# bad-samaritan/Polmux

Measured on AMD Instinct MI355X. Metric: dual-pol Gsample/s through SSFM+Rx-DSP, higher is better.
Workload: dtype f64

## Files before the change

### include/polmux_hip.h

```cpp
#ifndef POLMUX_HIP_H
#define POLMUX_HIP_H

#include <stddef.h>
#include <stdint.h>

#ifdef __cplusplus
extern "C" {
#endif

#define PLX_OK 0
#define PLX_ERR_HIP (-1)
#define PLX_ERR_ARG (-2)
#define PLX_ERR_UNSUPPORTED (-3)
#define PLX_ERR_REFERENCE (-4)
#define PLX_ERR_TIMEOUT (-5)

const char *plx_last_error(void);
int plx_abi_version(void);
int plx_device_count(int *count);
int plx_set_device(int device);

int plx_release_all(void);
int plx_gateway_stats(int64_t *out);
int plx_gateway_stats_ex(int64_t *out, int n);
// ... 6 lines not shown
    int32_t nfc;
    int32_t dual_pol;
    int32_t max_frames;
    int32_t fls[4];
    double dzmaxt;
    double dphimaxt;
    double alphalin;
    double length;
    int32_t nplates;
    int32_t manakov;
    const double *gam;
    const double *betat;
    const double *db1;
} plx_ssfm_desc;

typedef struct plx_ssfm plx_ssfm;

int plx_ssfm_create(plx_ssfm **plan, const plx_ssfm_desc *desc);
#define PLX_SSFM_SHARE_DEVICE 1u
#define PLX_SSFM_XPM_MANAKOV 2u
int plx_ssfm_create_ex(plx_ssfm **plan, const plx_ssfm_desc *desc, uint32_t flags);
typedef struct plx_ssfm_tuning {
    uint32_t size;
    int32_t no_fuse;
    int32_t short_rows;
    int32_t no_row_split;
    int32_t p1, logW;
    int32_t col_threads;
    int32_t rowr;
    int32_t rowsm;
    int32_t row256_split, row4k_split, rowg_split;
    int32_t no_pmd_tab;
    int32_t store_late;
    int32_t row_rev;
    int32_t safe_landing;
    int32_t reserved_[4];
    double barrier_timeout_ms;
} plx_ssfm_tuning;
int plx_ssfm_tuning_defaults(plx_ssfm_tuning *tuning);
int plx_ssfm_tuning_override(const plx_ssfm_tuning *tuning);
int plx_ssfm_create_tuned(plx_ssfm **plan, const plx_ssfm_desc *desc, uint32_t flags, const plx_ssfm_tuning *tuning);
int plx_ssfm_destroy(plx_ssfm *plan);
int plx_ssfm_set_birefringence(plx_ssfm *plan, const double *db0, const double *theta,
                               const double *epsilon, int nsets);
int plx_ssfm_set_birefringence_dev(plx_ssfm *plan, const double *db0, const double *theta,
                                   const double *epsilon, int nsets, void *stream);
int plx_ssfm_propagate_dev(plx_ssfm *plan, double *d_ux, double *d_uy, int nframes, void *stream);
int plx_ssfm_set_step_sequence(plx_ssfm *plan, const double *dz, int nsteps);
int plx_ssfm_log_steps(plx_ssfm *plan, int max_steps);
int plx_ssfm_step_sequence(plx_ssfm *plan, int frame, double *dz, int max_steps);
int plx_ssfm_results(plx_ssfm *plan, int nframes, double *firstdz, int32_t *ncycle);
int plx_ssfm_stats(plx_ssfm *plan, int64_t *row_pass_launches, int64_t *sample_steps);
int plx_ssfm_utilisation(plx_ssfm *plan, int64_t *frame_steps, int64_t *slots_listed, int64_t *slots_launched);
int plx_ssfm_info(plx_ssfm *plan, int32_t *info);
int plx_ssfm_barrier_timeouts(plx_ssfm *plan, int32_t *count, int rearm);
int plx_ssfm_profile(plx_ssfm *plan, int enable);
int plx_ssfm_kernel_times(plx_ssfm *plan, double *ms, int64_t *launches);

int plx_matrix_ssfm(double *uxr, double *uxi, double *uyr, double *uyi, const plx_ssfm_desc *desc,
                    const double *db0, const double *theta, const double *epsilon,
                    double *firstdz, int32_t *ncycle);
int plx_scalar_ssfm(double *ur, double *ui, const plx_ssfm_desc *desc, double *firstdz, int32_t *ncycle);
int plx_scalar_ssfm_adaptive(double *ur, double *ui, const plx_ssfm_desc *desc, int tolflag, double ltol,
                             double safety, double *firstdz, int32_t *ncycle, int32_t *nrej);

typedef struct plx_cde plx_cde;
int plx_cde_create(plx_cde **plan, int64_t fft_len, int64_t L, const double *H_interleaved);
int plx_cde_create_wdm(plx_cde **plan, int64_t fft_len, int64_t L, const double *H_interleaved, int32_t nch,
                       int32_t rows_per_channel);
int plx_cde_destroy(plx_cde *plan);
int plx_cde_apply_dev(plx_cde *plan, const double *d_x, double *d_y, int64_t nx, int nsig, void *stream);
int plx_cde_ofde(const double *xr, const double *xi, const double *yr, const double *yi, int64_t nx,
                 double fs, double lambda_ref, double span, double D, double S, int64_t fft_len,
                 int64_t L, double *oxr, double *oxi, double *oyr, double *oyi);

typedef struct plx_dbp_desc {
    int64_t nfft;
    int32_t max_frames;
    int32_t nspans;
    int32_t nsteps;
    int32_t manakov;
    double span_length;
    double alphalin;
    double gam;
    double xi;
    const double *betat;
    const double *dz;
} plx_dbp_desc;
typedef struct plx_dbp_plan plx_dbp_plan;
#define PLX_DBP_STREAMED 1u
int plx_dbp_create(plx_dbp_plan **plan, const plx_dbp_desc *desc, uint32_t flags);
int plx_dbp_destroy(plx_dbp_plan *plan);
int plx_dbp_apply_dev(plx_dbp_plan *plan, const double *d_in, double *d_out, int nframes, const double *d_scale, void *stream);
int plx_dbp(const double *xr, const double *xi, const double *yr, const double *yi, int64_t nx, const plx_dbp_desc *desc,
            double scale, double *oxr, double *oxi, double *oyr, double *oyi);

int plx_cmaadaptivefilter(const double *xr, const double *xi, int32_t Mdim, double *h1r, double *h1i,
                          double *h2r, double *h2i, double Ntap, double mu, const double *R, double sps,
                          double *yr, double *yi);
int plx_easiadaptivefilter(const double *xr, const double *xi, int32_t Mdim, double *h1r, double *h1i,
                           double *h2r, double *h2i, double Ntap, double mu, double sps, double *yr,
                           double *yi);

int plx_cmaadaptivefilter_m(const double *xr, const double *xi, int32_t Mdim, double *h1r, double *h1i,
                            double *h2r, double *h2i, int32_t ntap, double mu, const double *R, double *yr, double *yi);
int plx_easiadaptivefilter_m(const double *xr, const double *xi, int32_t Mdim, double *h1r, double *h1i,
// ... 131 lines not shown
```

### polmux_amd/_abi.py

```python
import ctypes as C
import os

_HERE = os.path.dirname(os.path.abspath(__file__))
LIB_PATH = os.path.join(_HERE, "lib", "libpolmux_hip.so")

PLX_OK = 0
PLX_ERR_HIP = -1
PLX_ERR_ARG = -2
PLX_ERR_UNSUPPORTED = -3
PLX_ERR_REFERENCE = -4
PLX_ERR_TIMEOUT = -5
PLX_SSFM_SHARE_DEVICE = 1
PLX_SSFM_XPM_MANAKOV = 2
PLX_DBP_STREAMED = 1
PLX_PHASE_TX = 2
PLX_PHASE_LO = 3
PLX_PHILOX_TX_DATA = 4
PLX_PHILOX_LO_DETUNE = 5


class PolmuxError(RuntimeError):
    def __init__(self, code, msg):
        super().__init__(msg)
        self.code = code
# ... 16 lines not shown

class DspParams(C.Structure):
    _fields_ = [("workatbaudrate", C.c_int32), ("applynlr", C.c_int32), ("nlralpha", C.c_double),
                ("power_mw", C.c_double), ("applypol", C.c_int32), ("polmethod", C.c_int32),
                ("cma_R", C.c_double * 2), ("cma_mu", C.c_double), ("cma_taps", C.c_int32),
                ("cma_txpolars", C.c_int32), ("cma_phizero", C.c_double), ("easi_mu", C.c_double),
                ("easi_txpolars", C.c_int32), ("easi_phizero", C.c_double), ("modorder", C.c_int32),
                ("freqavg", C.c_int32), ("phasavg", C.c_int32), ("poworder", C.c_int32),
                ("cma_has_mat", C.c_int32), ("easi_has_mat", C.c_int32), ("cma_mat", C.c_double * 8),
                ("easi_mat", C.c_double * 8), ("mfile_twins", C.c_int32), ("reserved_", C.c_int32)]


class FrontDesc(C.Structure):
    _fields_ = [("nfft", C.c_int64), ("dual_pol", C.c_int32), ("max_frames", C.c_int32), ("balanced", C.c_int32),
                ("adcbits", C.c_int32), ("decim", C.c_int32), ("ntaps", C.c_int32), ("fir", C.c_void_p),
                ("hopt_re", C.c_void_p), ("hopt_im", C.c_void_p), ("hel_re", C.c_void_p), ("hel_im", C.c_void_p),
                ("elo_re", C.c_void_p), ("elo_im", C.c_void_p), ("elo_scalar", C.c_double)]


class DbpDesc(C.Structure):
    _fields_ = [("nfft", C.c_int64), ("max_frames", C.c_int32), ("nspans", C.c_int32), ("nsteps", C.c_int32),
                ("manakov", C.c_int32), ("span_length", C.c_double), ("alphalin", C.c_double), ("gam", C.c_double),
                ("xi", C.c_double), ("betat", C.c_void_p), ("dz", C.c_void_p)]


_vp, _i32, _i64, _dbl, _sz = C.c_void_p, C.c_int32, C.c_int64, C.c_double, C.c_size_t

SIGNATURES = {
    "plx_abi_version": [],
    "plx_device_count": [C.POINTER(C.c_int)],
    "plx_set_device": [C.c_int],
    "plx_release_all": [],
    "plx_gateway_stats": [_vp],
    "plx_gateway_stats_ex": [_vp, C.c_int],
    "plx_fastexp": [_vp, _vp, _vp, _sz],
    "plx_fastexp_dev": [_vp, _vp, _sz, _vp],
    "plx_ssfm_create": [C.POINTER(_vp), C.POINTER(SsfmDesc)],
    "plx_ssfm_create_ex": [C.POINTER(_vp), C.POINTER(SsfmDesc), C.c_uint32],
    "plx_ssfm_tuning_defaults": [C.POINTER(SsfmTuning)],
    "plx_ssfm_tuning_override": [C.POINTER(SsfmTuning)],
    "plx_ssfm_create_tuned": [C.POINTER(_vp), C.POINTER(SsfmDesc), C.c_uint32, C.POINTER(SsfmTuning)],
    "plx_ssfm_destroy": [_vp],
    "plx_ssfm_set_step_sequence": [_vp, _vp, C.c_int],
    "plx_ssfm_log_steps": [_vp, C.c_int],
    "plx_ssfm_step_sequence": [_vp, C.c_int, _vp, C.c_int],
    "plx_ssfm_set_birefringence": [_vp, _vp, _vp, _vp, C.c_int],
    "plx_ssfm_set_birefringence_dev": [_vp, _vp, _vp, _vp, C.c_int, _vp],
    "plx_ssfm_propagate_dev": [_vp, _vp, _vp, C.c_int, _vp],
    "plx_ssfm_results": [_vp, C.c_int, _vp, _vp],
    "plx_ssfm_stats": [_vp, C.POINTER(_i64), C.POINTER(_i64)],
    "plx_ssfm_info": [_vp, _vp],
    "plx_ssfm_utilisation": [_vp, C.POINTER(_i64), C.POINTER(_i64), C.POINTER(_i64)],
    "plx_ssfm_barrier_timeouts": [_vp, C.POINTER(_i32), C.c_int],
    "plx_ssfm_profile": [_vp, C.c_int],
    "plx_ssfm_kernel_times": [_vp, _vp, _vp],
    "plx_matrix_ssfm": [_vp, _vp, _vp, _vp, C.POINTER(SsfmDesc), _vp, _vp, _vp, C.POINTER(_dbl),
                        C.POINTER(_i32)],
    "plx_scalar_ssfm": [_vp, _vp, C.POINTER(SsfmDesc), C.POINTER(_dbl), C.POINTER(_i32)],
    "plx_scalar_ssfm_adaptive": [_vp, _vp, C.POINTER(SsfmDesc), C.c_int, _dbl, _dbl, C.POINTER(_dbl), C.POINTER(_i32),
                                 C.POINTER(_i32)],
    "plx_cde_create": [C.POINTER(_vp), _i64, _i64, _vp],
    "plx_cde_create_wdm": [C.POINTER(_vp), _i64, _i64, _vp, _i32, _i32],
    "plx_cde_destroy": [_vp],
    "plx_cde_apply_dev": [_vp, _vp, _vp, _i64, C.c_int, _vp],
    "plx_cde_ofde": [_vp, _vp, _vp, _vp, _i64, _dbl, _dbl, _dbl, _dbl, _dbl, _i64, _i64, _vp, _vp, _vp, _vp],
    "plx_dbp_create": [C.POINTER(_vp), C.POINTER(DbpDesc), C.c_uint32],
    "plx_dbp_destroy": [_vp],
    "plx_dbp_apply_dev": [_vp, _vp, _vp, C.c_int, _vp, _vp],
    "plx_dbp": [_vp, _vp, _vp, _vp, _i64, C.POINTER(DbpDesc), _dbl, _vp, _vp, _vp, _vp],
    "plx_cmaadaptivefilter": [_vp, _vp, _i32, _vp, _vp, _vp, _vp, _dbl, _dbl, _vp, _dbl, _vp, _vp],
    "plx_easiadaptivefilter": [_vp, _vp, _i32, _vp, _vp, _vp, _vp, _dbl, _dbl, _dbl, _vp, _vp],
    "plx_cmaadaptivefilter_m": [_vp, _vp, _i32, _vp, _vp, _vp, _vp, _i32, _dbl, _vp, _vp, _vp],
    "plx_easiadaptivefilter_m": [_vp, _vp, _i32, _vp, _vp, _vp, _vp, _i32, _dbl, _vp, _vp],
    "plx_cmapolardemux": [_vp, _vp, _i64, _i32, _dbl, _vp, _vp, _vp, _vp, _vp, _vp, _vp, _vp, _vp],
    "plx_easipolardemux": [_vp, _vp, _i64, _dbl, _vp, _i32, _vp, _vp, _vp, _vp, _vp, _vp, _vp],
    "plx_poldemux_dev": [C.c_int, _vp, _vp, _i64, C.c_int, _i32, _dbl, _vp, _vp, _vp, _vp, _vp],
    "plx_dsp_create": [C.POINTER(_vp), _i64, _i32, _i32, C.POINTER(DspParams)],
    "plx_dsp_destroy": [_vp],
    "plx_dsp_run_dev": [_vp, _vp, _vp, C.c_int, _vp],
    "plx_dsp_run_freq_dev": [_vp, _vp, _vp, C.c_int, _vp, _vp],
    "plx_dsp_out_len": [_vp],
    "plx_decide_count_dev": [_vp, _i64, _i32, C.c_int, _vp, _vp, _vp, _vp],
    "plx_decide_count_frames_dev": [_vp, _i64, _i32, C.c_int, _vp, _i64, _vp, _vp, _vp],
    "plx_evm_dev": [_vp, _i64, _i32, C.c_int, _vp, _vp],
    "plx_decide_count_dqpsk_dev": [_vp, _i64, _i32, C.c_int, _vp, _i64, _vp, _vp],
    "plx_ampliflat_dev": [_vp, _vp, _i64, _i32, C.c_int, _dbl, _vp, _vp, C.c_uint64, _vp, _i32, _i32, _vp],
    "plx_phase_noise_dev": [_vp, _vp, _i64, _i64, _dbl, _i64, _i32, C.c_int, _vp, C.c_uint64, _vp, _i32, _vp, _vp, _vp,
                            _vp],
    "plx_lo_detune_dev": [_vp, _vp, _i64, _i64, _dbl, _i64, _i32, C.c_int, _i64, _i64, C.c_uint64, _vp, _vp, _vp, _i32, _vp,
                          _vp],
    "plx_tx_qpsk_dev": [_vp, _vp, _i64, _i32, _i32, C.c_int, _vp, _dbl, C.c_uint64, _vp, _vp, _vp, _vp, _vp],
    "plx_wdm_mux_dev": [_vp, _vp, _vp, _vp, _i64, _i32, C.c_int, _vp, _vp],
    "plx_wdm_select_dev": [_vp, _vp, _vp, _vp, _i64, _i32, C.c_int, _vp, _vp, _vp],
    "plx_pick_wdm_dev": [_vp, _vp, _vp, _i64, _i64, _i64, _dbl, _i32, C.c_int, _vp, _vp],
    "plx_front_create": [C.POINTER(_vp), C.POINTER(FrontDesc)],
    "plx_front_destroy": [_vp],
    "plx_front_out_len": [_vp],
    "plx_front_run_dev": [_vp, _vp, _vp, C.c_int, _vp, _vp, _vp],
    "plx_front_run_lo_dev": [_vp, _vp, _vp, C.c_int, _vp, _vp, _vp, _vp],
    "plx_rx_front": [_vp, _vp, _vp, _vp, C.POINTER(FrontDesc), _vp, _vp, _vp, _vp, _vp],
    "plx_filter_create": [C.POINTER(_vp), _i64, C.c_int, _vp, _vp],
    "plx_filter_destroy": [_vp],
    "plx_filter_apply_dev": [_vp, _vp, C.c_int, _vp],
    "plx_tx_bandlimit_dev": [_vp, _vp, _vp, C.c_int, _dbl, _vp, _vp, _vp],
    "plx_pmdinv_create": [C.POINTER(_vp), _i64, C.c_int],
    "plx_pmdinv_destroy": [_vp],
# ... 61 lines not shown
```

### polmux_amd/csrc/ssfm_plan.h

```cpp
#pragma once
#include "ssfm_kernels.h"
#include <vector>

using plxs::FrameCtl;
using plxs::SsfmArgs;

enum RowFamily { ROW_GENERAL, ROW_SM, ROW_256, ROW_REG, ROW_4K };
struct RowPass {
    plxs::sweep_kernel_t kern = nullptr;
    RowFamily family = ROW_GENERAL;
    unsigned threads = 0;
    unsigned gx = 0;
    size_t lds = 0;
    bool fold = false;
    bool single = false;
    bool twice = false;
};
enum RowUse {
    ROW_STEP,
    ROW_TABLE,
    ROW_MATRIX,
    ROW_USES
};

struct plx_ssfm {
    plx_ssfm_desc d;
    int p, p1, p2;
    size_t N;
    SsfmArgs a;
    double *d_betat = nullptr, *d_db1 = nullptr, *d_gam = nullptr, *d_brf = nullptr, *d_psum = nullptr;
    cplx *d_tpass = nullptr, *d_tw1 = nullptr, *d_tw2 = nullptr, *d_ctab = nullptr;
    FrameCtl *d_ctl = nullptr;
    unsigned long long *d_umax = nullptr;
    int *d_ndone = nullptr;
    int *h_ndone = nullptr;
    int *d_active = nullptr;
    hipEvent_t ev = nullptr;
    std::vector<FrameCtl> h_ctl;
    int brf_sets = 0;
    size_t lds_col = 0;
    cplx *d_e1 = nullptr, *d_e2 = nullptr;
    unsigned long long *d_slots = nullptr;
    unsigned long long *d_mbox = nullptr;
    size_t mbox_bytes = 0;
    int fused = 0, fused_grid = 0, tiles_pf = 0;
    uint32_t flags = 0;
    int xpm_dual = 0;
    int barrier_timeouts = 0;
    int calls_unfused = 0, rearm_after = 16;
    double *d_dzlist = nullptr, *d_dzlog = nullptr;
    int dzlist_cap = 0;
    int col_threads = 512;
    RowPass row[ROW_USES];
    cplx *d_tw2c = nullptr, *d_twmid = nullptr;
    int tw_compact = 0;
    double *h_brf[2] = {nullptr, nullptr};
    hipEvent_t brf_ev[2] = {nullptr, nullptr};
    int brf_slot = 0;
    int64_t row_launches = 0, sample_steps = 0;
    int64_t slots_launched = 0, slots_listed = 0, frame_steps = 0;
    int profile = 0;
    struct ProfRun { std::vector<hipEvent_t> ev; std::vector<int> cls, step; int maxnc = 0; bool fused = false; };
    std::vector<hipEvent_t> evfree;
    std::vector<ProfRun> prof_pending;
    double k_ms[4] = {0, 0, 0, 0};
    int64_t k_launches[4] = {0, 0, 0, 0};
};

PLX_HIDDEN int plx_ssfm_linear_dev(plx_ssfm *P, const SsfmArgs &base, cplx *d_x, double dz, hipStream_t st);

static const double kInv2Pi = 0.15915494309189533577;
```

### polmux_amd/csrc/ssfm_plan.hip

```cpp
#include "ssfm_plan.h"
#include "ssfm_ctrl.h"
#include "plx_gateway.h"

#include <cmath>
#include <cstdlib>
#include <cstring>
#include <limits>
#include <vector>
using namespace plxs;

static int ilog2(int64_t v)
{
    int l = 0;
    while (((int64_t)1 << l) < v) l++;
    return l;
}

static void free_plan(plx_ssfm *P)
{
    if (!P) return;
    hipFree(P->d_betat); hipFree(P->d_db1); hipFree(P->d_gam); hipFree(P->d_brf); hipFree(P->d_psum);
    hipFree(P->d_tpass); hipFree(P->d_tw1); hipFree(P->d_tw2); hipFree(P->d_ctab); hipFree(P->d_ctl); hipFree(P->d_umax);
    hipFree(P->d_dzlist); hipFree(P->d_dzlog); hipFree(P->d_tw2c); hipFree(P->d_twmid);
    hipFree(P->d_ndone); hipFree(P->d_slots); hipFree(P->d_mbox); hipFree(P->d_active); hipFree(P->d_e1); hipFree(P->d_e2);
    if (P->h_ndone) hipHostFree(P->h_ndone);
    if (P->ev) hipEventDestroy(P->ev);
    for (hipEvent_t e : P->evfree) hipEventDestroy(e);
    for (auto &r : P->prof_pending) for (hipEvent_t e : r.ev) hipEventDestroy(e);
    for (int k = 0; k < 2; k++) {
        if (P->h_brf[k]) hipHostFree(P->h_brf[k]);
        if (P->brf_ev[k]) hipEventDestroy(P->brf_ev[k]);
    }
    delete P;
}

static cplx phasor(uint64_t e, int64_t M)
{
    const long double ang = -2.0L * 3.14159265358979323846264338327950288L * (long double)e / (long double)M;
    return make_double2((double)cosl(ang), (double)sinl(ang));
}

static std::vector<cplx> half_table(int M)
{
    std::vector<cplx> t(M / 2 > 0 ? M / 2 : 1);
    for (int k = 0; k < M / 2; k++) t[k] = phasor(k, M);
    return t;
}

static std::vector<cplx> compact_table(int M)
{
    std::vector<cplx> t(M / 8 + 4);
    for (int k = 0; k < M / 8 + 4; k++) t[k] = phasor(k < M / 8 ? 4 * k : k - M / 8, M);
    return t;
}

static std::vector<cplx> mid_table(int R)
{
    std::vector<cplx> tm(7 * 16, make_double2(1.0, 0.0));
    for (int j = 0; j < 16; j++) {
        if (R == 2) tm[j] = phasor(j, 32);
        const int q0 = R == 8 ? 4 : 0;
        if (R >= 4) for (int q = 0; q < 3; q++) tm[16 * (q0 + q) + j] = phasor((q + 1) * j, 64);
        if (R == 8) for (int q = 0; q < 4; q++) tm[16 * q + j] = phasor(j + 16 * q, 128);
    }
    return tm;
}


namespace {
plx_ssfm_tuning g_override;
bool g_have_override = false;
}

extern "C" int plx_ssfm_tuning_defaults(plx_ssfm_tuning *t)
{
    if (!t) PLX_FAIL(PLX_ERR_ARG, "plx_ssfm_tuning_defaults: null argument");
    std::memset(t, 0, sizeof(*t));
    t->size = (uint32_t)sizeof(*t);
    t->p1 = -1; t->logW = -1; t->col_threads = -1; t->store_late = -1;
    t->row_rev = 1; t->rowr = 1; t->rowsm = 1; t->row256_split = 1; t->row4k_split = 1; t->rowg_split = 1;
    t->barrier_timeout_ms = 500.0;
    if (const char *e = getenv("PLX_SSFM_NO_FUSE")) t->no_fuse = atoi(e);
    if (const char *e = getenv("PLX_SSFM_BARRIER_TIMEOUT_MS")) t->barrier_timeout_ms = atof(e);
    return PLX_OK;
}

extern "C" int plx_ssfm_tuning_override(const plx_ssfm_tuning *t)
{
    if (t && t->size != sizeof(plx_ssfm_tuning)) PLX_FAIL(PLX_ERR_ARG, "plx_ssfm_tuning_override: fill the struct with plx_ssfm_tuning_defaults first");
    g_have_override = t != nullptr;
    if (t) g_override = *t;
    return PLX_OK;
}

static bool resolve_rows(plx_ssfm *P, const plx_ssfm_tuning &tune)
{
    const SsfmArgs &a = P->a;
    const int N1 = 1 << a.p1, N2 = 1 << a.p2, npol = a.dual ? 2 : 1;
    const bool dual = a.dual != 0, pmd = a.pmd != 0, tab = a.e1tab != nullptr;
    RowPass *const row = P->row;
    auto pass = [](sweep_kernel_t k, RowFamily family, int gx, int threads, size_t lds) { return RowPass{k, family, (unsigned)threads, (unsigned)gx, lds}; };
    auto upload = [](cplx *&dst, const std::vector<cplx> &v) {
        return hipMalloc((void **)&dst, v.size() * sizeof(cplx)) == hipSuccess &&
               hipMemcpy(dst, v.data(), v.size() * sizeof(cplx), hipMemcpyHostToDevice) == hipSuccess;
    };
    if (P->tw_compact) {
        if (allow_lds(row4k_kernel(false, false), ROW4K_LDS(false, false)) != hipSuccess || allow_lds(row4k_kernel(true, false), ROW4K_LDS(true, false)) != hipSuccess ||
            allow_lds(row4k_kernel(false, true), ROW4K_LDS(false, false)) != hipSuccess) return false;
        const bool split = tune.row4k_split != 0;
        RowPass one = pass(row4k_kernel(false, split), ROW_4K, N1 * npol, 256, ROW4K_LDS(false, split));
        RowPass both = pass(row4k_kernel(true, false), ROW_4K, N1, 512, ROW4K_LDS(true, false));
        one.fold = both.fold = true;
        one.single = dual;
        row[ROW_STEP] = pmd ? both : one; row[ROW_TABLE] = one; row[ROW_MATRIX] = both;
        return true;
    }
    int rowthr = ROW_THREADS;
    while (rowthr < 1024 && (int64_t)rowthr * 8 < (int64_t)npol * a.R * N2) rowthr *= 2;
    const RowPass whole = pass(row_kernel(), ROW_GENERAL, N1 / a.R, rowthr, ROW_LDS(npol * a.R, N2));
    RowPass halves = pass(row_kernel(), ROW_GENERAL, N1, N2 / 8 < ROW_THREADS ? ROW_THREADS : (N2 / 8 > 1024 ? 1024 : N2 / 8), ROW_LDS(1, N2));
    halves.single = halves.twice = true;
    const bool row_split = dual && N2 >= 2048 && !tune.no_row_split;
    if (allow_lds(row_kernel(), row_split && halves.lds > whole.lds ? halves.lds : whole.lds) != hipSuccess) return false;
    row[ROW_STEP] = row[ROW_TABLE] = row[ROW_MATRIX] = whole;
    if (row_split) { row[ROW_TABLE] = halves; if (!pmd) row[ROW_STEP] = halves; }

    const int rowsm_min = dual ? (tune.rowsm == 2 ? 5 : 7) : 5, per_wave = 64 / (N2 / 16);
    if (tune.rowr && tune.rowsm && !pmd && a.p2 >= rowsm_min && a.p2 <= 7 && (N1 * npol) % per_wave == 0) {
        if (!upload(P->d_twmid, mid_table(N2 / 16))) return false;
        if (allow_lds(rowsm_kernel(a.p2, !dual), ROWSM_LDS) == hipSuccess)
            row[ROW_STEP] = row[ROW_TABLE] = pass(rowsm_kernel(a.p2, !dual), ROW_SM, N1 * npol / per_wave, ROWR_THREADS, ROWSM_LDS);
    }
    if (tune.rowr && a.p1 == 8 && a.p2 == 8) {
        if (!dual) {
            if (allow_lds(row256_kernel(false, true, false), ROWR_LDS_SC) == hipSuccess)
                row[ROW_STEP] = pass(row256_kernel(false, true, false), ROW_256, 64, ROWR_THREADS, ROWR_LDS_SC);
        } else if (allow_lds(row256_kernel(pmd, false, false), ROWR_LDS) == hipSuccess) {
            row[ROW_STEP] = pass(row256_kernel(pmd, false, false), ROW_256, 128, ROWR_THREADS, ROWR_LDS);
            if (pmd && tune.row256_split && allow_lds(row256_kernel(true, false, true), ROWR_LDS) == hipSuccess && tab)
                row[ROW_STEP] = pass(row256_kernel(true, false, true), ROW_256, 128, ROWR_THREADS, ROWR_LDS_SPLIT);
        }
    }
    const int rows_wg = ROWG_THREADS / (N2 / 16) / npol;
// ... 79 lines not shown
        free_plan(P);
        PLX_FAIL(PLX_ERR_UNSUPPORTED, "plx_ssfm_create: 4096-point rows need the one-polarisation row pass (PLX_SSFM_NO_ROW_SPLIT is set)");
    }
    a.spm = desc->fls[2]; a.xpm = desc->fls[3]; a.manakov = desc->manakov ? 1 : 0; a.pmd = desc->fls[1] ? 1 : 0;
    a.nplates = desc->nplates;
    a.alphalin = desc->alphalin; a.Lf = desc->length; a.dzmax = desc->dzmaxt; a.dphimax = desc->dphimaxt;
    a.lcorr = desc->length / desc->nplates;
    a.invN = 1.0 / (double)N;
    a.spin_ticks = (long long)(tune.barrier_timeout_ms * 1e5);
    a.safe_land = tune.safe_landing;
    a.row_rev = tune.row_rev;
    if ((int64_t)desc->max_frames + 4 >= ((int64_t)1 << 22)) { free_plan(P); PLX_FAIL(PLX_ERR_UNSUPPORTED, "plx_ssfm_create: max_frames must be below 2^22 - 4"); }

    std::vector<double> bt((size_t)nfc * N), d1;
    std::vector<cplx> tp((size_t)N);
    const bool have_db1 = desc->db1 != nullptr && a.dual;
    if (have_db1) d1.resize((size_t)nfc * N);
    for (int j = 0; j < N1; j++) {
        const unsigned k1 = plx_bitrev((unsigned)j, P->p1);
        for (int i = 0; i < N2; i++) {
            const unsigned k2 = plx_bitrev((unsigned)i, P->p2);
            const size_t k = (size_t)k1 + (size_t)N1 * k2, pos = (size_t)j * N2 + i;
            for (int c = 0; c < nfc; c++) {
                bt[(size_t)c * N + pos] = desc->betat[(size_t)c * N + k] * kInv2Pi;
                if (have_db1) d1[(size_t)c * N + pos] = desc->db1[(size_t)c * N + k] * kInv2Pi;
            }
            tp[pos] = phasor(((uint64_t)i * k1) & (uint64_t)(N - 1), N);
        }
    }
    const std::vector<cplx> t1 = half_table(N1), t2 = P->tw_compact ? compact_table(N2) : half_table(N2);
    std::vector<double> gam(nfc);
    for (int c = 0; c < nfc; c++) gam[c] = (a.dual && a.manakov) ? desc->gam[c] * 8 / 9 : desc->gam[c];

#define UP(dst, vec, T)                                                                             \
    do {                                                                                            \
        if (hipMalloc((void **)&(dst), (vec).size() * sizeof(T)) != hipSuccess ||                   \
            hipMemcpy((dst), (vec).data(), (vec).size() * sizeof(T), hipMemcpyHostToDevice) != hipSuccess) { \
            free_plan(P);                                                                           \
            PLX_FAIL(PLX_ERR_HIP, "plx_ssfm_create: device allocation/upload failed");              \
        }                                                                                           \
    } while (0)
    UP(P->d_betat, bt, double);
    if (have_db1) UP(P->d_db1, d1, double);
    UP(P->d_tpass, tp, cplx);
    UP(P->d_tw1, t1, cplx);
    UP(P->d_tw2, t2, cplx);
    {
        std::vector<cplx> ctv(PLX_CTAB);
        for (int k = 0; k < PLX_CTAB; k++) ctv[k] = phasor(k, PLX_CTAB);
        UP(P->d_ctab, ctv, cplx);
    }
    UP(P->d_gam, gam, double);
#undef UP
    bool ok = hipMalloc((void **)&P->d_ctl, sizeof(FrameCtl) * F) == hipSuccess &&
              hipMalloc((void **)&P->d_umax, sizeof(unsigned long long) * F * nfc) == hipSuccess &&
              hipMalloc((void **)&P->d_ndone, 64) == hipSuccess &&
              hipMalloc((void **)&P->d_active, sizeof(int) * (size_t)F) == hipSuccess &&
              hipHostMalloc((void **)&P->h_ndone, 64, hipHostMallocDefault) == hipSuccess &&
              hipEventCreateWithFlags(&P->ev, hipEventDisableTiming) == hipSuccess;
    if (ok && !a.dual && a.xpm) ok = hipMalloc((void **)&P->d_psum, sizeof(double) * (size_t)F * N) == hipSuccess;
    P->xpm_dual = xpm_dual ? 1 : 0;
    if (ok && xpm_dual) ok = hipMalloc((void **)&P->d_psum, sizeof(double) * 4 * (size_t)F * N) == hipSuccess;
    if (!ok) { free_plan(P); PLX_FAIL(PLX_ERR_HIP, "plx_ssfm_create: device allocation failed"); }
    a.betat_p = P->d_betat; a.db1_p = P->d_db1; a.tpass = P->d_tpass; a.tw1 = P->d_tw1; a.tw2 = P->d_tw2; a.ctab = P->d_ctab;
    a.gam = P->d_gam; a.ctl = P->d_ctl; a.umax = P->d_umax; a.ndone = P->d_ndone; a.psum = P->d_psum;
    P->h_ctl.resize(F);

    P->lds_col = (((size_t)N1 << a.logT) + N1 / 2) * sizeof(cplx) + 32 * sizeof(double) + 8 * sizeof(FrameCtl) + 128 + COLX_NFC * sizeof(double) + 128 * sizeof(cplx);
    P->col_threads = P->lds_col > 80 * 1024 ? 1024 : 512;
    if (tune.col_threads == 128 || tune.col_threads == 256 || tune.col_threads == 512 || tune.col_threads == 1024) P->col_threads = tune.col_threads;
    if (allow_lds(colx16_kernel(true), P->lds_col) != hipSuccess || allow_lds(colx16_kernel(false), P->lds_col) != hipSuccess || allow_lds(col_fwd_kernel(), P->lds_col) != hipSuccess ||
        allow_lds(col_inv_kernel(), P->lds_col) != hipSuccess || (P->xpm_dual && allow_lds(col_fwd_xpm_kernel(), P->lds_col) != hipSuccess)) {
        free_plan(P);
        PLX_FAIL(PLX_ERR_HIP, "plx_ssfm_create: cannot reserve LDS for the transform kernels");
    }
    if (((a.dual && a.W == 8) || (!a.dual && a.W == 16 && !desc->fls[3])) && !tune.no_fuse && a.p1 == 8 && nfc <= COLX_NFC) {
        int ncu = 256;
        {
            int dev = 0, v = 0;
            if (hipGetDevice(&dev) == hipSuccess && hipDeviceGetAttribute(&v, hipDeviceAttributeMultiprocessorCount, dev) == hipSuccess && v > 0)
                ncu = v;
        }
        const int tiles_pf = nfc * (N2 / a.W);
        const int per_cu = blocks_per_cu(colx16_kernel(a.dual != 0), 256, P->lds_col);
        const int cap = ncu * per_cu;
        if (tiles_pf <= cap) {
            P->fused = 1;
            P->tiles_pf = tiles_pf;
            P->fused_grid = (cap / tiles_pf) * tiles_pf;
            a.store_late = tune.store_late >= 0 ? (tune.store_late ? 1 : 0) : (P->fused_grid > tiles_pf ? 1 : 0);
            const int mstride = F + 4;
            P->mbox_bytes = sizeof(unsigned long long) * ((size_t)mstride * (P->fused_grid / tiles_pf) + 1);
            if (hipMalloc((void **)&P->d_slots, sizeof(unsigned long long) * 2 * (size_t)F * tiles_pf) != hipSuccess ||
                hipMalloc((void **)&P->d_mbox, P->mbox_bytes) != hipSuccess) {
                free_plan(P);
                PLX_FAIL(PLX_ERR_HIP, "plx_ssfm_create: device allocation failed");
            }
            a.slots = P->d_slots;
            a.mbox = P->d_mbox;
            a.mbox_stride = mstride;
            a.grab = (int *)(P->d_mbox + (size_t)mstride * (P->fused_grid / tiles_pf));
        }
    }
    if (a.pmd && have_db1 && !tune.no_pmd_tab) {
        const double D = desc->db1[1] * kInv2Pi;
        bool lin = D != 0.0 && N >= 4;
        for (int c = 0; c < nfc && lin; c++)
            for (int64_t k = 0; k < N && lin; k++) {
                const double m = (double)(k < N / 2 ? k : k - N);
                if (fabs(desc->db1[(size_t)c * N + k] * kInv2Pi - D * m) > 4e-15 * fabs(D) * (double)N) lin = false;
            }
        if (lin) {
            const int tmax = (int)ceil(desc->dzmaxt / a.lcorr) + 2;
            const size_t n1 = (size_t)F * tmax * N1, n2 = (size_t)F * tmax * N2;
            if (tmax <= 64 && (n1 + n2) * sizeof(cplx) <= ((size_t)4 << 30)) {
                if (hipMalloc((void **)&P->d_e1, n1 * sizeof(cplx)) != hipSuccess || hipMalloc((void **)&P->d_e2, n2 * sizeof(cplx)) != hipSuccess) {
// ... 61 lines not shown
}

extern "C" int plx_ssfm_set_birefringence(plx_ssfm *P, const double *db0, const double *theta,
                                          const double *epsilon, int nsets)
{
    return set_brf(P, db0, theta, epsilon, nsets, nullptr, true);
}

extern "C" int plx_ssfm_set_birefringence_dev(plx_ssfm *P, const double *db0, const double *theta,
                                              const double *epsilon, int nsets, void *stream)
{
    return set_brf(P, db0, theta, epsilon, nsets, (hipStream_t)stream, false);
}

static void launch_row(plx_ssfm *P, const SsfmArgs &a, unsigned FC, hipStream_t st, RowUse use)
{
    const RowPass &r = P->row[use];
    const dim3 g = r.fold ? dim3(r.gx * FC) : dim3(r.gx, FC), bs(r.threads);
    if (!r.single) { launch(r.kern, g, bs, r.lds, st, a); return; }
    SsfmArgs b = a;
    b.dual = 0; b.R = 1; b.logR = 0;
    launch(r.kern, g, bs, r.lds, st, b);
    if (r.twice) { b.ux = a.uy; launch(r.kern, g, bs, r.lds, st, b); }
}

static int resolve_profiles(plx_ssfm *P)
{
    for (auto &r : P->prof_pending) {
        for (size_t i = 0; i + 1 < r.ev.size(); i++) {
            const int cls = r.cls[i], step = r.step[i];
            const bool active = (r.fused && cls == 0) ? step <= r.maxnc : step < r.maxnc;
            if (!active) continue;
            float ms = 0;
            PLX_HIP(hipEventElapsedTime(&ms, r.ev[i], r.ev[i + 1]));
            P->k_ms[cls] += ms;
            P->k_launches[cls]++;
        }
        for (hipEvent_t e : r.ev) P->evfree.push_back(e);
    }
    P->prof_pending.clear();
    return PLX_OK;
}

static int propagate_frames(plx_ssfm *P, cplx *d_ux, cplx *d_uy, int nframes, hipStream_t st)
{
    SsfmArgs a = P->a;
    const int nfc = a.nfc, N2 = 1 << a.p2;
    a.ux = d_ux;
    a.uy = d_uy;
    a.nframes = nframes;
    a.active = P->d_active;
    a.nactive = P->d_ndone + 2;
    unsigned FC = (unsigned)nframes * nfc;
    PLX_HIP(hipMemsetAsync(a.ctl, 0, sizeof(FrameCtl) * nframes, st));
    PLX_HIP(hipMemsetAsync(a.umax, 0, sizeof(unsigned long long) * FC, st));
    PLX_HIP(hipMemsetAsync(P->d_ndone, 0, 64, st));
    const bool fused = P->fused != 0;
    if (fused) {
        PLX_HIP(hipMemsetAsync(P->d_slots, 0xFF, sizeof(unsigned long long) * 2 * (size_t)nframes * P->tiles_pf, st));
        PLX_HIP(hipMemsetAsync(P->d_mbox, 0, P->mbox_bytes, st));
    } else {
        unsigned gx = (unsigned)((P->N + 255) / 256);
        if (gx > 64) gx = 64;
        launch_umax(dim3(gx, FC), st, a);
    }
    const dim3 blk(256);
    const dim3 bcol((unsigned)P->col_threads);
    const bool compact_every_step = nframes >= 64;
    int chunk = 4, steps = 0;
    const int kMaxSteps = 1 << 19;
    bool pending = false, aborted = false;
    struct ProfGuard {
        plx_ssfm *P;
        plx_ssfm::ProfRun run;
        ~ProfGuard() { for (hipEvent_t e : run.ev) P->evfree.push_back(e); }
    } guard{P, {}};
    plx_ssfm::ProfRun &run = guard.run;
    auto mark = [&](int cls, int step) -> int {
        if (!P->profile) return PLX_OK;
        hipEvent_t e;
        if (!P->evfree.empty()) { e = P->evfree.back(); P->evfree.pop_back(); }
        else PLX_HIP(hipEventCreate(&e));
        run.ev.push_back(e); run.cls.push_back(cls); run.step.push_back(step);
        PLX_HIP(hipEventRecord(e, st));
        return PLX_OK;
    };
#define PLX_MARK(cls, step) do { int rc_ = mark((cls), (step)); if (rc_) return rc_; } while (0)
    for (;;) {
        for (int sidx = 0; sidx < chunk; sidx++) {
            const dim3 gcol((unsigned)(N2 / a.W), FC);
            P->slots_launched += FC / nfc;
            if (fused) {
                const int tcx = (int)gcol.x, tct = (int)(gcol.x * FC);
                const dim3 gx((unsigned)(tct < P->fused_grid ? tct : P->fused_grid));
                if (compact_every_step || sidx == 0) {
                    PLX_MARK(3, steps + sidx);
                    launch_compact(a.ctl, nframes, P->d_active, P->d_ndone + 2, compact_every_step ? 1 : chunk, st);
                }
#ifdef PLX_EMU
                emu::g_concurrency = emu::starve_barriers() ? 1 : P->tiles_pf;
#endif
                a.round = steps + sidx;
                PLX_MARK(0, steps + sidx);
                launch(colx16_kernel(a.dual != 0), gx, blk, P->lds_col, st, a, tcx, P->tiles_pf);
#ifdef PLX_EMU
                emu::g_concurrency = 1;
#endif
                if (a.e1tab) {
                    PLX_MARK(3, steps + sidx);
                    launch_pmd_tab(FC / nfc, st, a);
                }
                PLX_MARK(1, steps + sidx);
                launch_row(P, a, FC, st, ROW_STEP);
                P->row_launches++;
                continue;
            }
            PLX_MARK(3, steps + sidx);
            launch_ctrl(nframes, st, a);
            if (compact_every_step || sidx == 0)
                launch_compact(a.ctl, nframes, P->d_active, P->d_ndone + 2, compact_every_step ? 1 : chunk, st);
            if (!a.dual && a.xpm) {
                unsigned gx = (unsigned)((P->N + 255) / 256);
                if (gx > 256) gx = 256;
                launch_rowsum(dim3(gx, (unsigned)nframes), st, a);
            }
            if (P->xpm_dual) {
                unsigned gx = (unsigned)((P->N + 255) / 256);
                if (gx > 256) gx = 256;
                launch_stokes_sum(dim3(gx, (unsigned)nframes), st, a);
            }
            if (a.e1tab) launch_pmd_tab(FC / nfc, st, a);
            PLX_MARK(0, steps + sidx);
            launch(P->xpm_dual ? col_fwd_xpm_kernel() : col_fwd_kernel(), gcol, bcol, P->lds_col, st, a);
            PLX_MARK(1, steps + sidx);
            launch_row(P, a, FC, st, ROW_STEP);
            PLX_MARK(2, steps + sidx);
            launch(col_inv_kernel(), gcol, bcol, P->lds_col, st, a);
            P->row_launches++;
        }
        PLX_MARK(3, steps + chunk);
        if (steps == 0 && !P->prof_pending.empty()) {
            const int rc_ = resolve_profiles(P);
            if (rc_) return rc_;
        }
        steps += chunk;
        if (pending) {
            PLX_HIP(hipEventSynchronize(P->ev));
            if (P->h_ndone[1]) { aborted = true; break; }
            if (P->h_ndone[0] >= nframes) break;
            const unsigned live = (unsigned)(nframes - P->h_ndone[0]) * nfc;
            if (live < FC) FC = live;
        }
        PLX_HIP(hipMemcpyAsync(P->h_ndone, P->d_ndone, 4 * sizeof(int), hipMemcpyDeviceToHost, st));
        PLX_HIP(hipEventRecord(P->ev, st));
        pending = true;
        if (chunk > 8) chunk = 4;
        else if (chunk < (compact_every_step ? 8 : 16)) chunk *= 2;
        if (steps > kMaxSteps) PLX_FAIL(PLX_ERR_HIP, "plx_ssfm_propagate_dev: step loop did not terminate");
    }
    PLX_HIP(hipMemcpyAsync(P->h_ctl.data(), a.ctl, sizeof(FrameCtl) * nframes, hipMemcpyDeviceToHost, st));
    PLX_HIP(hipMemcpyAsync(P->h_ndone, P->d_ndone, 4 * sizeof(int), hipMemcpyDeviceToHost, st));
    PLX_HIP(hipStreamSynchronize(st));
    P->slots_listed += P->h_ndone[3];
    if (aborted || P->h_ndone[1]) {
        P->barrier_timeouts++;
        P->fused = 0;
        PLX_FAIL(PLX_ERR_TIMEOUT, "plx_ssfm_propagate_dev: frame barrier timed out (the workgroups of a frame were not co-resident: "
                                  "another kernel holds the GPU); nothing was stored after the time-out and the field of this call is "
                                  "INVALID -- the plan now takes the barrier-free three-sweep step: restore the field and call again, "
                                  "or create such plans with plx_ssfm_create_ex(..., PLX_SSFM_SHARE_DEVICE)");
    }
    int maxnc = 0;
    for (int f = 0; f < nframes; f++) {
        P->frame_steps += P->h_ctl[f].ncycle + (fused ? 1 : 0);
        if (!P->h_ctl[f].done) PLX_FAIL(PLX_ERR_HIP, "plx_ssfm_propagate_dev: a frame did not reach the fibre end");
        P->sample_steps += (int64_t)P->h_ctl[f].ncycle * (int64_t)P->N * nfc;
        if (P->h_ctl[f].ncycle > maxnc) maxnc = P->h_ctl[f].ncycle;
    }
    if (!run.ev.empty()) {
        run.maxnc = maxnc; run.fused = fused;
        P->prof_pending.push_back(std::move(run));
        run.ev.clear();
    }
#undef PLX_MARK
    return PLX_OK;
}

extern "C" int plx_ssfm_propagate_dev(plx_ssfm *P, double *d_ux, double *d_uy, int nframes, void *stream)
{
    if (!P || !d_ux) PLX_FAIL(PLX_ERR_ARG, "plx_ssfm_propagate_dev: null argument");
    if (nframes < 1 || nframes > P->d.max_frames) PLX_FAIL(PLX_ERR_ARG, "plx_ssfm_propagate_dev: nframes out of range");
    if (P->a.dual && !d_uy) PLX_FAIL(PLX_ERR_ARG, "plx_ssfm_propagate_dev: dual-polarisation plan needs d_uy");
    if (P->a.brf_per_frame && P->brf_sets < nframes)
        PLX_FAIL(PLX_ERR_ARG, "plx_ssfm_propagate_dev: fewer birefringence sets than frames");
    P->slots_launched = 0; P->slots_listed = 0; P->row_launches = 0; P->sample_steps = 0; P->frame_steps = 0;
    const int rc = propagate_frames(P, (cplx *)d_ux, (cplx *)d_uy, nframes, (hipStream_t)stream);
    if (rc) return rc;
    PLX_HIP(hipGetLastError());
    return PLX_OK;
}

extern "C" int plx_ssfm_set_step_sequence(plx_ssfm *P, const double *dz, int nsteps)
{
    if (!P || nsteps < 0 || (nsteps > 0 && !dz)) PLX_FAIL(PLX_ERR_ARG, "plx_ssfm_set_step_sequence: bad argument");
    if (nsteps > P->dzlist_cap) {
        if (P->d_dzlist) { (void)hipFree(P->d_dzlist); P->d_dzlist = nullptr; P->dzlist_cap = 0; }
        PLX_HIP(hipMalloc((void **)&P->d_dzlist, sizeof(double) * (size_t)nsteps));
        P->dzlist_cap = nsteps;
    }
    if (nsteps > 0) PLX_HIP(hipMemcpy(P->d_dzlist, dz, sizeof(double) * (size_t)nsteps, hipMemcpyHostToDevice));
    P->a.dzlist = nsteps > 0 ? P->d_dzlist : nullptr;
    P->a.ndz = nsteps;
    return PLX_OK;
}

extern "C" int plx_ssfm_log_steps(plx_ssfm *P, int max_steps)
{
    if (!P || max_steps < 0) PLX_FAIL(PLX_ERR_ARG, "plx_ssfm_log_steps: bad argument");
    if (P->d_dzlog) { (void)hipFree(P->d_dzlog); P->d_dzlog = nullptr; }
    P->a.dzlog = nullptr; P->a.logcap = 0;
    if (max_steps > 0) {
        PLX_HIP(hipMalloc((void **)&P->d_dzlog, sizeof(double) * (size_t)max_steps * P->d.max_frames));
        P->a.dzlog = P->d_dzlog; P->a.logcap = max_steps;
    }
    return PLX_OK;
}

extern "C" int plx_ssfm_step_sequence(plx_ssfm *P, int frame, double *dz, int max_steps)
{
    if (!P || !dz || frame < 0 || frame >= P->d.max_frames || max_steps < 0) PLX_FAIL(PLX_ERR_ARG, "plx_ssfm_step_sequence: bad argument");
    if (!P->d_dzlog) PLX_FAIL(PLX_ERR_ARG, "plx_ssfm_step_sequence: no log (plx_ssfm_log_steps)");
    const int n = max_steps < P->a.logcap ? max_steps : P->a.logcap;
    PLX_HIP(hipMemcpy(dz, P->d_dzlog + (size_t)frame * P->a.logcap, sizeof(double) * (size_t)n, hipMemcpyDeviceToHost));
    return PLX_OK;
}

extern "C" int plx_ssfm_utilisation(plx_ssfm *P, int64_t *frame_steps, int64_t *slots_listed, int64_t *slots_launched)
{
    if (!P) PLX_FAIL(PLX_ERR_ARG, "plx_ssfm_utilisation: null plan");
    if (frame_steps) *frame_steps = P->frame_steps;
    if (slots_listed) *slots_listed = P->slots_listed;
    if (slots_launched) *slots_launched = P->slots_launched;
    return PLX_OK;
}

extern "C" int plx_ssfm_info(plx_ssfm *P, int32_t *info)
{
    if (!P || !info) PLX_FAIL(PLX_ERR_ARG, "plx_ssfm_info: null argument");
    info[0] = P->fused; info[1] = P->p1; info[2] = P->p2; info[3] = P->fused_grid; info[4] = P->tiles_pf;
    info[5] = P->col_threads;
    const RowPass &s = P->row[ROW_STEP], &t = P->row[ROW_TABLE];
    info[6] = (int32_t)(s.family == ROW_GENERAL ? t.threads : s.threads);
    info[7] = (s.family == ROW_SM || s.family == ROW_REG) ? 2 : s.family == ROW_4K ? ((P->a.dual && !s.single) ? 0 : 1) : (t.twice ? 1 : 0);
    return PLX_OK;
}

extern "C" int plx_ssfm_barrier_timeouts(plx_ssfm *P, int32_t *count, int rearm)
{
    if (!P) PLX_FAIL(PLX_ERR_ARG, "plx_ssfm_barrier_timeouts: null plan");
    if (count) *count = P->barrier_timeouts;
    if (rearm && !P->fused && P->fused_grid > 0 && P->tiles_pf > 0) { P->fused = 1; P->calls_unfused = 0; }
    return PLX_OK;
}

extern "C" int plx_ssfm_profile(plx_ssfm *P, int enable)
{
    if (!P) PLX_FAIL(PLX_ERR_ARG, "plx_ssfm_profile: null plan");
    P->profile = enable ? 1 : 0;
    return PLX_OK;
}

extern "C" int plx_ssfm_kernel_times(plx_ssfm *P, double *ms, int64_t *launches)
{
    if (!P || !ms || !launches) PLX_FAIL(PLX_ERR_ARG, "plx_ssfm_kernel_times: null argument");
    const int rc = resolve_profiles(P);
    if (rc) return rc;
    for (int k = 0; k < 4; k++) { ms[k] = P->k_ms[k]; launches[k] = P->k_launches[k]; P->k_ms[k] = 0; P->k_launches[k] = 0; }
    return PLX_OK;
}

int plx_ssfm_filter_table(plx_ssfm *P, const double *h_re, const double *h_im, cplx **d_out)
{
    if (!P || !h_re || !d_out) PLX_FAIL(PLX_ERR_ARG, "filter table: null argument");
    const int N1 = 1 << P->p1, N2 = 1 << P->p2;
    std::vector<cplx> h(P->N);
    for (int j = 0; j < N1; j++) {
        const unsigned k1 = plx_bitrev((unsigned)j, P->p1);
        for (int i = 0; i < N2; i++) {
            const size_t k = (size_t)k1 + (size_t)N1 * plx_bitrev((unsigned)i, P->p2);
            h[(size_t)j * N2 + i] = make_double2(h_re[k], h_im ? h_im[k] : 0.0);
        }
    }
    cplx *d = nullptr;
    if (hipMalloc((void **)&d, P->N * sizeof(cplx)) != hipSuccess ||
        hipMemcpy(d, h.data(), P->N * sizeof(cplx), hipMemcpyHostToDevice) != hipSuccess) {
        if (d) (void)hipFree(d);
        PLX_FAIL(PLX_ERR_HIP, "filter table: device allocation/upload failed");
    }
    *d_out = d;
    return PLX_OK;
}

void plx_ssfm_geometry(const plx_ssfm *P, int *p1, int *p2) { *p1 = P->p1; *p2 = P->p2; }

int plx_ssfm_filter_dev(plx_ssfm *P, cplx *d_ux, cplx *d_uy, const cplx *d_hmul, int nframes, void *stream, const cplx *d_umat)
{
    if (!P || !d_ux || (!d_hmul && !d_umat)) PLX_FAIL(PLX_ERR_ARG, "filter: null argument");
    if (d_umat && (!P->a.dual || P->a.nfc != 1)) PLX_FAIL(PLX_ERR_ARG, "filter: matrix tables need a dual-polarisation single-field plan");
    if (nframes < 1 || nframes > P->d.max_frames) PLX_FAIL(PLX_ERR_ARG, "filter: nframes outside [1, max_frames]");
    if (P->a.dual && !d_uy) PLX_FAIL(PLX_ERR_ARG, "filter: dual-polarisation plan needs d_uy");
    hipStream_t st = (hipStream_t)stream;
    SsfmArgs b = P->a;
    b.ux = d_ux; b.uy = d_uy; b.nframes = nframes; b.hmul = d_hmul; b.umat = d_umat;
    b.force = 1; b.spm = 0; b.xpm = 0; b.pmd = 0; b.f_cur = 0; b.f_leff = 0; b.f_sc = b.invN;
// ... 45 lines not shown
```

Measured before the change: 0.6660.

## Plan SSFM step loop from previous call's cycle counts; merge control memsets

Each propagate call remembers the frame count, the min/max step cycles and the fused mode. The next matching call uses them to clip the final chunk at the expected end, so the host can finish after one sync. It also skips per-step compaction launches until frames are expected to leave the active set. The control, umax and ndone buffers move into one allocation so they can be cleared with a single memset. If a call deviates from the expectation it falls back to short chunks; this adds a host round-trip and keeps history state in the plan.

```diff
diff --git a/include/polmux_hip.h b/include/polmux_hip.h
--- a/include/polmux_hip.h
+++ b/include/polmux_hip.h
@@ -82,6 +82,8 @@
 int plx_ssfm_results(plx_ssfm *plan, int nframes, double *firstdz, int32_t *ncycle);
 int plx_ssfm_stats(plx_ssfm *plan, int64_t *row_pass_launches, int64_t *sample_steps);
 int plx_ssfm_utilisation(plx_ssfm *plan, int64_t *frame_steps, int64_t *slots_listed, int64_t *slots_launched);
+int plx_ssfm_loop_stats(plx_ssfm *plan, int64_t out[4]);
+int plx_ssfm_expectation(plx_ssfm *plan, int on);
 int plx_ssfm_info(plx_ssfm *plan, int32_t *info);
 int plx_ssfm_barrier_timeouts(plx_ssfm *plan, int32_t *count, int rearm);
 int plx_ssfm_profile(plx_ssfm *plan, int enable);
diff --git a/polmux_amd/_abi.py b/polmux_amd/_abi.py
--- a/polmux_amd/_abi.py
+++ b/polmux_amd/_abi.py
@@ -92,6 +92,8 @@
     "plx_ssfm_info": [_vp, _vp],
     "plx_ssfm_utilisation": [_vp, C.POINTER(_i64), C.POINTER(_i64), C.POINTER(_i64)],
     "plx_ssfm_barrier_timeouts": [_vp, C.POINTER(_i32), C.c_int],
+    "plx_ssfm_loop_stats": [_vp, _vp],
+    "plx_ssfm_expectation": [_vp, C.c_int],
     "plx_ssfm_profile": [_vp, C.c_int],
     "plx_ssfm_kernel_times": [_vp, _vp, _vp],
     "plx_matrix_ssfm": [_vp, _vp, _vp, _vp, C.POINTER(SsfmDesc), _vp, _vp, _vp, C.POINTER(_dbl),
diff --git a/polmux_amd/csrc/ssfm_plan.h b/polmux_amd/csrc/ssfm_plan.h
--- a/polmux_amd/csrc/ssfm_plan.h
+++ b/polmux_amd/csrc/ssfm_plan.h
@@ -32,6 +32,7 @@
     cplx *d_tpass = nullptr, *d_tw1 = nullptr, *d_tw2 = nullptr, *d_ctab = nullptr;
     FrameCtl *d_ctl = nullptr;
     unsigned long long *d_umax = nullptr;
+    size_t ctl_bytes = 0;
     int *d_ndone = nullptr;
     int *h_ndone = nullptr;
     int *d_active = nullptr;
@@ -59,6 +60,10 @@
     int brf_slot = 0;
     int64_t row_launches = 0, sample_steps = 0;
     int64_t slots_launched = 0, slots_listed = 0, frame_steps = 0;
+    struct Expect { int frames = 0, minnc = 0, maxnc = 0, fused = 0; } expect;
+    unsigned tune_gen = 0;
+    int expect_on = 1;
+    int64_t loop_stats[4] = {0, 0, 0, 0};
     int profile = 0;
     struct ProfRun { std::vector<hipEvent_t> ev; std::vector<int> cls, step; int maxnc = 0; bool fused = false; };
     std::vector<hipEvent_t> evfree;
diff --git a/polmux_amd/csrc/ssfm_plan.hip b/polmux_amd/csrc/ssfm_plan.hip
--- a/polmux_amd/csrc/ssfm_plan.hip
+++ b/polmux_amd/csrc/ssfm_plan.hip
@@ -20,9 +20,9 @@
 {
     if (!P) return;
     hipFree(P->d_betat); hipFree(P->d_db1); hipFree(P->d_gam); hipFree(P->d_brf); hipFree(P->d_psum);
-    hipFree(P->d_tpass); hipFree(P->d_tw1); hipFree(P->d_tw2); hipFree(P->d_ctab); hipFree(P->d_ctl); hipFree(P->d_umax);
+    hipFree(P->d_tpass); hipFree(P->d_tw1); hipFree(P->d_tw2); hipFree(P->d_ctab); hipFree(P->d_ctl);
     hipFree(P->d_dzlist); hipFree(P->d_dzlog); hipFree(P->d_tw2c); hipFree(P->d_twmid);
-    hipFree(P->d_ndone); hipFree(P->d_slots); hipFree(P->d_mbox); hipFree(P->d_active); hipFree(P->d_e1); hipFree(P->d_e2);
+    hipFree(P->d_slots); hipFree(P->d_mbox); hipFree(P->d_active); hipFree(P->d_e1); hipFree(P->d_e2);
     if (P->h_ndone) hipHostFree(P->h_ndone);
     if (P->ev) hipEventDestroy(P->ev);
     for (hipEvent_t e : P->evfree) hipEventDestroy(e);
@@ -70,6 +70,7 @@
 namespace {
 plx_ssfm_tuning g_override;
 bool g_have_override = false;
+unsigned g_tune_gen = 0;
 }
 
 extern "C" int plx_ssfm_tuning_defaults(plx_ssfm_tuning *t)
@@ -81,7 +82,13 @@
     t->row_rev = 1; t->rowr = 1; t->rowsm = 1; t->row256_split = 1; t->row4k_split = 1; t->rowg_split = 1;
     t->barrier_timeout_ms = 500.0;
     if (const char *e = getenv("PLX_SSFM_NO_FUSE")) t->no_fuse = atoi(e);
-    if (const char *e = getenv("PLX_SSFM_BARRIER_TIMEOUT_MS")) t->barrier_timeout_ms = atof(e);
+    if (const char *e = getenv("PLX_SSFM_BARRIER_TIMEOUT_MS")) {
+        char *end = nullptr;
+        const double v = strtod(e, &end);
+        while (end && (*end == ' ' || *end == '\t')) end++;
+        if (end != e && *end == '\0' && std::isfinite(v) && v >= 1.0 && v <= 60000.0) t->barrier_timeout_ms = v;
+        else plx_set_error(std::string("plx_ssfm_tuning_defaults: PLX_SSFM_BARRIER_TIMEOUT_MS=\"") + e + "\" is not a time in [1, 60000] ms: the frame barrier keeps 500 ms");
+    }
     return PLX_OK;
 }
 
@@ -89,6 +96,7 @@
 {
     if (t && t->size != sizeof(plx_ssfm_tuning)) PLX_FAIL(PLX_ERR_ARG, "plx_ssfm_tuning_override: fill the struct with plx_ssfm_tuning_defaults first");
     g_have_override = t != nullptr;
+    g_tune_gen++;
     if (t) g_override = *t;
     return PLX_OK;
 }
@@ -274,9 +282,9 @@
     }
     UP(P->d_gam, gam, double);
 #undef UP
-    bool ok = hipMalloc((void **)&P->d_ctl, sizeof(FrameCtl) * F) == hipSuccess &&
-              hipMalloc((void **)&P->d_umax, sizeof(unsigned long long) * F * nfc) == hipSuccess &&
-              hipMalloc((void **)&P->d_ndone, 64) == hipSuccess &&
+    const size_t umax_off = sizeof(FrameCtl) * (size_t)F, ndone_off = (umax_off + sizeof(unsigned long long) * (size_t)F * nfc + 63) / 64 * 64;
+    P->ctl_bytes = ndone_off + 64;
+    bool ok = hipMalloc((void **)&P->d_ctl, P->ctl_bytes) == hipSuccess &&
               hipMalloc((void **)&P->d_active, sizeof(int) * (size_t)F) == hipSuccess &&
               hipHostMalloc((void **)&P->h_ndone, 64, hipHostMallocDefault) == hipSuccess &&
               hipEventCreateWithFlags(&P->ev, hipEventDisableTiming) == hipSuccess;
@@ -284,6 +292,8 @@
     P->xpm_dual = xpm_dual ? 1 : 0;
     if (ok && xpm_dual) ok = hipMalloc((void **)&P->d_psum, sizeof(double) * 4 * (size_t)F * N) == hipSuccess;
     if (!ok) { free_plan(P); PLX_FAIL(PLX_ERR_HIP, "plx_ssfm_create: device allocation failed"); }
+    P->d_umax = (unsigned long long *)((char *)P->d_ctl + umax_off);
+    P->d_ndone = (int *)((char *)P->d_ctl + ndone_off);
     a.betat_p = P->d_betat; a.db1_p = P->d_db1; a.tpass = P->d_tpass; a.tw1 = P->d_tw1; a.tw2 = P->d_tw2; a.ctab = P->d_ctab;
     a.gam = P->d_gam; a.ctl = P->d_ctl; a.umax = P->d_umax; a.ndone = P->d_ndone; a.psum = P->d_psum;
     P->h_ctl.resize(F);
@@ -451,10 +461,20 @@
     a.active = P->d_active;
     a.nactive = P->d_ndone + 2;
     unsigned FC = (unsigned)nframes * nfc;
-    PLX_HIP(hipMemsetAsync(a.ctl, 0, sizeof(FrameCtl) * nframes, st));
-    PLX_HIP(hipMemsetAsync(a.umax, 0, sizeof(unsigned long long) * FC, st));
-    PLX_HIP(hipMemsetAsync(P->d_ndone, 0, 64, st));
+    if (P->ctl_bytes <= ((size_t)1 << 20) || nframes == P->d.max_frames) {
+        PLX_HIP(hipMemsetAsync(a.ctl, 0, P->ctl_bytes, st));
+    } else {
+        PLX_HIP(hipMemsetAsync(a.ctl, 0, sizeof(FrameCtl) * nframes, st));
+        PLX_HIP(hipMemsetAsync(a.umax, 0, sizeof(unsigned long long) * FC, st));
+        PLX_HIP(hipMemsetAsync(P->d_ndone, 0, 64, st));
+    }
     const bool fused = P->fused != 0;
+    const bool diag = a.dzlist != nullptr || a.dzlog != nullptr;
+    const plx_ssfm::Expect want = P->expect;
+    P->expect = plx_ssfm::Expect();
+    const bool have_exp = P->expect_on && !diag && P->tune_gen == g_tune_gen && want.frames == nframes && want.fused == (fused ? 1 : 0);
+    const int exp_rounds = have_exp ? want.maxnc + 1 : 0, exp_leave = have_exp ? want.minnc - 1 : 0;
+    for (int k = 0; k < 4; k++) P->loop_stats[k] = 0;
     if (fused) {
         PLX_HIP(hipMemsetAsync(P->d_slots, 0xFF, sizeof(unsigned long long) * 2 * (size_t)nframes * P->tiles_pf, st));
         PLX_HIP(hipMemsetAsync(P->d_mbox, 0, P->mbox_bytes, st));
@@ -466,6 +486,8 @@
     const dim3 blk(256);
     const dim3 bcol((unsigned)P->col_threads);
     const bool compact_every_step = nframes >= 64;
+    bool seen_leave = false, clipped_end = false, missed = false;
+    int64_t rebuilds = 0;
     int chunk = 4, steps = 0;
     const int kMaxSteps = 1 << 19;
     bool pending = false, aborted = false;
@@ -486,15 +508,28 @@
     };
 #define PLX_MARK(cls, step) do { int rc_ = mark((cls), (step)); if (rc_) return rc_; } while (0)
     for (;;) {
+        const bool clip = have_exp && !missed && steps < exp_rounds && steps + chunk >= exp_rounds;
+        if (clip) chunk = exp_rounds - steps;
+        auto rebuild = [&](int sidx) {
+            if (sidx == 0) return true;
+            if (!compact_every_step) return false;
+            return !have_exp || seen_leave || steps + sidx >= exp_leave;
+        };
+        auto serves = [&](int sidx) {
+            int n = 1;
+            while (sidx + n < chunk && !rebuild(sidx + n)) n++;
+            return n;
+        };
         for (int sidx = 0; sidx < chunk; sidx++) {
             const dim3 gcol((unsigned)(N2 / a.W), FC);
             P->slots_launched += FC / nfc;
             if (fused) {
                 const int tcx = (int)gcol.x, tct = (int)(gcol.x * FC);
                 const dim3 gx((unsigned)(tct < P->fused_grid ? tct : P->fused_grid));
-                if (compact_every_step || sidx == 0) {
+                if (rebuild(sidx)) {
                     PLX_MARK(3, steps + sidx);
-                    launch_compact(a.ctl, nframes, P->d_active, P->d_ndone + 2, compact_every_step ? 1 : chunk, st);
+                    launch_compact(a.ctl, nframes, P->d_active, P->d_ndone + 2, serves(sidx), st);
+                    rebuilds++;
                 }
 #ifdef PLX_EMU
                 emu::g_concurrency = emu::starve_barriers() ? 1 : P->tiles_pf;
@@ -516,8 +551,10 @@
             }
             PLX_MARK(3, steps + sidx);
             launch_ctrl(nframes, st, a);
-            if (compact_every_step || sidx == 0)
-                launch_compact(a.ctl, nframes, P->d_active, P->d_ndone + 2, compact_every_step ? 1 : chunk, st);
+            if (rebuild(sidx)) {
+                launch_compact(a.ctl, nframes, P->d_active, P->d_ndone + 2, serves(sidx), st);
+                rebuilds++;
+            }
             if (!a.dual && a.xpm) {
                 unsigned gx = (unsigned)((P->N + 255) / 256);
                 if (gx > 256) gx = 256;
@@ -543,23 +580,43 @@
             if (rc_) return rc_;
         }
         steps += chunk;
+        if (clip) {
+            PLX_HIP(hipMemcpyAsync(P->h_ctl.data(), a.ctl, sizeof(FrameCtl) * nframes, hipMemcpyDeviceToHost, st));
+            PLX_HIP(hipMemcpyAsync(P->h_ndone, P->d_ndone, 4 * sizeof(int), hipMemcpyDeviceToHost, st));
+            PLX_HIP(hipEventRecord(P->ev, st));
+            PLX_HIP(hipEventSynchronize(P->ev));
+            pending = false;
+            if (P->h_ndone[1]) { aborted = true; break; }
+            if (P->h_ndone[0] >= nframes) { clipped_end = true; break; }
+            const unsigned live = (unsigned)(nframes - P->h_ndone[0]) * nfc;
+            if (live < FC) FC = live;
+            if (P->h_ndone[0] > 0) seen_leave = true;
+            missed = true;
+            chunk = 2;
+            continue;
+        }
         if (pending) {
             PLX_HIP(hipEventSynchronize(P->ev));
             if (P->h_ndone[1]) { aborted = true; break; }
             if (P->h_ndone[0] >= nframes) break;
             const unsigned live = (unsigned)(nframes - P->h_ndone[0]) * nfc;
             if (live < FC) FC = live;
+            if (P->h_ndone[0] > 0) seen_leave = true;
         }
         PLX_HIP(hipMemcpyAsync(P->h_ndone, P->d_ndone, 4 * sizeof(int), hipMemcpyDeviceToHost, st));
         PLX_HIP(hipEventRecord(P->ev, st));
         pending = true;
-        if (chunk > 8) chunk = 4;
+        if (missed) chunk = 2;
+        else if (chunk > 8) chunk = 4;
         else if (chunk < (compact_every_step ? 8 : 16)) chunk *= 2;
         if (steps > kMaxSteps) PLX_FAIL(PLX_ERR_HIP, "plx_ssfm_propagate_dev: step loop did not terminate");
     }
-    PLX_HIP(hipMemcpyAsync(P->h_ctl.data(), a.ctl, sizeof(FrameCtl) * nframes, hipMemcpyDeviceToHost, st));
-    PLX_HIP(hipMemcpyAsync(P->h_ndone, P->d_ndone, 4 * sizeof(int), hipMemcpyDeviceToHost, st));
-    PLX_HIP(hipStreamSynchronize(st));
+    P->loop_stats[0] = steps; P->loop_stats[1] = rebuilds; P->loop_stats[2] = exp_rounds; P->loop_stats[3] = clipped_end ? 1 : 0;
+    if (!clipped_end) {
+        PLX_HIP(hipMemcpyAsync(P->h_ctl.data(), a.ctl, sizeof(FrameCtl) * nframes, hipMemcpyDeviceToHost, st));
+        PLX_HIP(hipMemcpyAsync(P->h_ndone, P->d_ndone, 4 * sizeof(int), hipMemcpyDeviceToHost, st));
+        PLX_HIP(hipStreamSynchronize(st));
+    }
     P->slots_listed += P->h_ndone[3];
     if (aborted || P->h_ndone[1]) {
         P->barrier_timeouts++;
@@ -569,12 +626,17 @@
                                   "INVALID -- the plan now takes the barrier-free three-sweep step: restore the field and call again, "
                                   "or create such plans with plx_ssfm_create_ex(..., PLX_SSFM_SHARE_DEVICE)");
     }
-    int maxnc = 0;
+    int maxnc = 0, minnc = std::numeric_limits<int>::max();
     for (int f = 0; f < nframes; f++) {
         P->frame_steps += P->h_ctl[f].ncycle + (fused ? 1 : 0);
         if (!P->h_ctl[f].done) PLX_FAIL(PLX_ERR_HIP, "plx_ssfm_propagate_dev: a frame did not reach the fibre end");
         P->sample_steps += (int64_t)P->h_ctl[f].ncycle * (int64_t)P->N * nfc;
         if (P->h_ctl[f].ncycle > maxnc) maxnc = P->h_ctl[f].ncycle;
+        if (P->h_ctl[f].ncycle < minnc) minnc = P->h_ctl[f].ncycle;
+    }
+    if (P->expect_on && !diag) {
+        P->expect.frames = nframes; P->expect.minnc = minnc; P->expect.maxnc = maxnc; P->expect.fused = fused ? 1 : 0;
+        P->tune_gen = g_tune_gen;
     }
     if (!run.ev.empty()) {
         run.maxnc = maxnc; run.fused = fused;
@@ -659,6 +721,22 @@
     if (!P) PLX_FAIL(PLX_ERR_ARG, "plx_ssfm_barrier_timeouts: null plan");
     if (count) *count = P->barrier_timeouts;
     if (rearm && !P->fused && P->fused_grid > 0 && P->tiles_pf > 0) { P->fused = 1; P->calls_unfused = 0; }
+    if (rearm) P->expect = plx_ssfm::Expect();
+    return PLX_OK;
+}
+
+extern "C" int plx_ssfm_loop_stats(plx_ssfm *P, int64_t *out)
+{
+    if (!P || !out) PLX_FAIL(PLX_ERR_ARG, "plx_ssfm_loop_stats: null argument");
+    for (int k = 0; k < 4; k++) out[k] = P->loop_stats[k];
+    return PLX_OK;
+}
+
+extern "C" int plx_ssfm_expectation(plx_ssfm *P, int on)
+{
+    if (!P) PLX_FAIL(PLX_ERR_ARG, "plx_ssfm_expectation: null plan");
+    P->expect_on = on ? 1 : 0;
+    P->expect = plx_ssfm::Expect();
     return PLX_OK;
 }
 
```

Result: no change. 0.6644 (-0.2%).
